# bytedance/particle-sfm

Measured on NVIDIA H100. Metric: global_ba_observations_per_sec, higher is better.
Workload: dtype f64

## Files before the change

particle-sfm_b200/csrc/ba_kernels.cuh:

```cuda
#pragma once
#include "psfm_common.cuh"

namespace psfm {
namespace ba {

constexpr int NVL = 18;
constexpr int NVI = 9;
constexpr int NREP = 32;

struct TileCtx {
  const int* tile_start;
  const int* tile_pt;
  const int* pt_ptr;
  const int* obs_img;
  const int* obs_pt;
  const unsigned short* obs_lseg;
  const unsigned short* obs_lpt;
  const double2* obs_xy;
  const unsigned short* tile_perm;
  const int* cseg_ptr;
  const int* cseg_img;
  const unsigned short* cseg_off;
  const int* img_cam;
  int F, P, M, C, T;
// ... 409 lines not shown
}

template <int TILE, bool ROT>
__global__ void __launch_bounds__(TILE, (TILE == 256 ? 3 : 1)) k_linearize(const TileCtx tc, const LinArgs a) {
  extern __shared__ __align__(16) unsigned char smem_raw[];
  TileSmem<TILE> sm;
  sm.carve(smem_raw, 18, 3, tc.cap_ns, tc.cap_np);
  const TileInfo ti = tile_header(tc);
  const int tid = threadIdx.x;
  const bool act = tid < ti.n;
  const size_t i = (size_t)ti.base + tid;
  int ls = 0, lp = 0;
  double2 xy = make_double2(0.0, 0.0);
  if (act) {
    ls = __ldg(tc.obs_lseg + i);
    lp = __ldg(tc.obs_lpt + i);
    xy = tc.obs_xy[i];
  }
  tile_fill_smem<TILE>(tc, sm, ti, a.pose16, nullptr, a.X, nullptr, nullptr, true);
  linearize_tile<TILE, ROT>(tc, a, sm, ti, act, ls, lp, xy, blockIdx.x);
}


struct PtsArgs {
  const double* hpp;
  const double* gp;
  const double* wk;
  const double* scale_p;
  double radius, min_diag, max_diag;
  int intr;
  int P;
  double* ht;
  double* wt;
  double* acc_intr;
  double* acc_fail;
  double* gmax;
};

__global__ void __launch_bounds__(256) k_point_blocks(const PtsArgs a) {
  __shared__ double sred[9 * 32];
  const int p = blockIdx.x * 256 + threadIdx.x;
  double gm = 0.0, fail = 0.0;
  double ci[9];
#pragma unroll
  for (int k = 0; k < 9; ++k) ci[k] = 0.0;
  if (p < a.P) {
    const size_t P = a.P;
    const double s0 = a.scale_p[3 * (size_t)p], s1 = a.scale_p[3 * (size_t)p + 1], s2 = a.scale_p[3 * (size_t)p + 2];
    double h00 = a.hpp[p] * s0 * s0, h01 = a.hpp[P + p] * s0 * s1, h02 = a.hpp[2 * P + p] * s0 * s2,
           h11 = a.hpp[3 * P + p] * s1 * s1, h12 = a.hpp[4 * P + p] * s1 * s2, h22 = a.hpp[5 * P + p] * s2 * s2;
    const double g0 = a.gp[p], g1 = a.gp[P + p], g2 = a.gp[2 * P + p];
    h00 += fmin(fmax(h00, a.min_diag), a.max_diag) / a.radius;
    h11 += fmin(fmax(h11, a.min_diag), a.max_diag) / a.radius;
    h22 += fmin(fmax(h22, a.min_diag), a.max_diag) / a.radius;
    bool bad = !(h00 > 0.0);
    const double l00 = sqrt(h00);
    const double l10 = h01 / l00, l20 = h02 / l00;
    double d = h11 - l10 * l10;
    bad |= !(d > 0.0);
    const double l11 = sqrt(d);
    const double l21 = (h12 - l20 * l10) / l11;
    d = h22 - l20 * l20 - l21 * l21;
    bad |= !(d > 0.0);
    const double l22 = sqrt(d);
    const double i00 = 1.0 / l00, i11 = 1.0 / l11, i22 = 1.0 / l22;
    const double i10 = -l10 * i00 * i11;
    const double i21 = -l21 * i11 * i22;
    const double i20 = -(l20 * i00 + l21 * i10) * i22;
    double v00 = i00 * i00 + i10 * i10 + i20 * i20, v01 = i10 * i11 + i20 * i21, v02 = i20 * i22,
           v11 = i11 * i11 + i21 * i21, v12 = i21 * i22, v22 = i22 * i22;
    if (bad) { fail = 1.0; v00 = v11 = v22 = 1.0; v01 = v02 = v12 = 0.0; }
    v00 *= s0 * s0; v01 *= s0 * s1; v02 *= s0 * s2; v11 *= s1 * s1; v12 *= s1 * s2; v22 *= s2 * s2;
    a.ht[p] = v00; a.ht[P + p] = v01; a.ht[2 * P + p] = v02;
    a.ht[3 * P + p] = v11; a.ht[4 * P + p] = v12; a.ht[5 * P + p] = v22;
    const double w0 = v00 * g0 + v01 * g1 + v02 * g2;
    const double w1 = v01 * g0 + v11 * g1 + v12 * g2;
    const double w2 = v02 * g0 + v12 * g1 + v22 * g2;
    a.wt[p] = w0; a.wt[P + p] = w1; a.wt[2 * P + p] = w2;
    gm = fmax(fmax(fabs(g0), fabs(g1)), fabs(g2));
    if (a.intr >= 1) {
      double W[3][3], WH[3][3];
      for (int j = 0; j < 3; ++j)
        for (int k = 0; k < 3; ++k) W[j][k] = (j < a.intr) ? a.wk[(size_t)(3 * j + k) * P + p] : 0.0;
      for (int j = 0; j < 3; ++j) {
        WH[j][0] = W[j][0] * v00 + W[j][1] * v01 + W[j][2] * v02;
        WH[j][1] = W[j][0] * v01 + W[j][1] * v11 + W[j][2] * v12;
        WH[j][2] = W[j][0] * v02 + W[j][1] * v12 + W[j][2] * v22;
      }
      int c = 0;
      for (int j = 0; j < 3; ++j)
        for (int k = j; k < 3; ++k) ci[c++] = -(WH[j][0] * W[k][0] + WH[j][1] * W[k][1] + WH[j][2] * W[k][2]);
      for (int j = 0; j < 3; ++j) ci[6 + j] = -(W[j][0] * w0 + W[j][1] * w1 + W[j][2] * w2);
    }
  }
  const double m = block_max(gm, sred);
  if (threadIdx.x == 0 && m > 0.0) atomic_max_nonneg(a.gmax, m);
  const double f = block_sum(fail, sred);
  if (threadIdx.x == 0 && f > 0.0) atomicAdd(a.acc_fail, f);
  if (a.intr >= 1) {
    const double s = block_sum_multi<9>(ci, sred);
    if (threadIdx.x < 9) atomicAdd(a.acc_intr + threadIdx.x, s);
  }
}

// ... 340 lines not shown
```

particle-sfm_b200/csrc/ba_schur_explicit.cuh:

```cuda
#pragma once
#include <cooperative_groups.h>
#include <cub/cub.cuh>

#include "ba_kernels.cuh"
#include "ba_tile_pipe.cuh"

namespace psfm {
namespace ba {

constexpr int NVX = 21;
constexpr int NVX2 = 27;


struct SwArgs {
  Lin L;
  const double* pose16;
  const double* X;
  const double* ht;
  const double* wk;
  const double* K;
  double* W;
  double* WH;
  double* acc_cam;
  size_t rep_stride;
// ... 122 lines not shown
    for (int k = 0; k < 36; ++k) acc[k] = 0.0;
    for (int e = rg.x; e < rg.y; ++e) {
      const unsigned int u = __ldg(a.entries + e);
      const size_t i = base + (u >> 16), j = base + (u & 0xffffu);
      const double2* wh = reinterpret_cast<const double2*>(a.WH + 18 * i);
      const double2* wj = reinterpret_cast<const double2*>(a.W + 18 * j);
      double A[18], B[18];
#pragma unroll
      for (int k = 0; k < 9; ++k) {
        const double2 x = __ldg(wh + k), y = __ldg(wj + k);
        A[2 * k] = x.x; A[2 * k + 1] = x.y;
        B[2 * k] = y.x; B[2 * k + 1] = y.y;
      }
#pragma unroll
      for (int r = 0; r < 6; ++r)
#pragma unroll
        for (int c = 0; c < 6; ++c)
          acc[6 * r + c] += A[3 * r] * B[3 * c] + A[3 * r + 1] * B[3 * c + 1] + A[3 * r + 2] * B[3 * c + 2];
    }
    double* dst = band + (size_t)__ldg(a.task_slot + q) * 36;
#pragma unroll
    for (int k = 0; k < 36; ++k)
      if (acc[k] != 0.0) atomicAdd(dst + k, acc[k]);
  }
}


constexpr int PS = 18;

struct StArgs {
  Lin L;
  const double* pose16;
  const double* X;
  const double* ht;
  const double* wt;
  const double* wk;
  const double* K;
  double* acc_cam;
  size_t rep_stride;
  int intr;
  const unsigned int* entries;
  const int* task_slot;
  const int2* task_rng;
  const int* tile_task;
  double* Sband;
  size_t band_stride;
  int nrep_mask;
  int span;
  const unsigned char* tile_dense;
};

enum : unsigned char { TILE_PAIRS_LOOP = 0, TILE_PAIRS_DENSE = 1, TILE_PAIRS_DENSE_DUP = 2 };

__host__ __device__ inline int dense_z_kb2(int np) { return (3 * np + 7) >> 3; }
__host__ __device__ inline int dense_z_rb(int ns) { return (6 * ns + 15) >> 4; }
__host__ __device__ inline size_t dense_z_doubles(int ns, int np) { return (size_t)dense_z_rb(ns) * dense_z_kb2(np) * 128; }

__device__ __forceinline__ void dmma_16x8x4(double (&d)[4], double a0, double a1, double b) {
  asm("mma.sync.aligned.m16n8k4.row.col.f64.f64.f64.f64 {%0,%1,%2,%3}, {%4,%5}, {%6}, {%0,%1,%2,%3};"
      : "+d"(d[0]), "+d"(d[1]), "+d"(d[2]), "+d"(d[3])
      : "d"(a0), "d"(a1), "d"(b));
}

__device__ __forceinline__ bool chol3(const double (&h)[6], double (&l)[6]) {
  const double d0 = h[0];
  l[0] = sqrt(d0);
  l[1] = h[1] / l[0];
  l[3] = h[2] / l[0];
  const double d1 = h[3] - l[1] * l[1];
  l[2] = sqrt(d1);
  l[4] = (h[4] - l[3] * l[1]) / l[2];
  const double d2 = h[5] - l[3] * l[3] - l[4] * l[4];
  l[5] = sqrt(d2);
  auto ok = [](double d) { return d > 0.0 && !isinf(d); };
  return ok(d0) && ok(d1) && ok(d2);
}

template <int TILE>
__device__ __forceinline__ void dense_pairs_mma(const double* __restrict__ zf, const int* __restrict__ cimg, int ns, int np,
                                                double* __restrict__ band, int span) {
  const int lane = threadIdx.x & 31, warp = threadIdx.x >> 5;
  const int R = 6 * ns, RB = dense_z_rb(ns), KB2 = dense_z_kb2(np);
  const int nblk = RB * (RB + 1) / 2;
  const double2* z2 = reinterpret_cast<const double2*>(zf);
  for (int blk = warp; blk < nblk; blk += TILE / 32) {
    int I = 0, rem = blk;
    while (rem >= RB - I) { rem -= RB - I; ++I; }
    const int J = I + rem;
    const double2* pa0 = z2 + (size_t)(2 * I) * KB2 * 32 + (lane ^ ((2 * I) & 7));
    const double2* pa1 = z2 + (size_t)(2 * I + 1) * KB2 * 32 + (lane ^ ((2 * I + 1) & 7));
    const double2* pb0 = z2 + (size_t)(2 * J) * KB2 * 32 + (lane ^ ((2 * J) & 7));
    const double2* pb1 = z2 + (size_t)(2 * J + 1) * KB2 * 32 + (lane ^ ((2 * J + 1) & 7));
    double acc[2][4];
#pragma unroll
    for (int h = 0; h < 2; ++h)
#pragma unroll
      for (int e = 0; e < 4; ++e) acc[h][e] = 0.0;
#pragma unroll 2
    for (int k = 0; k < KB2; ++k) {
      const double2 a0 = pa0[32 * k], a1 = pa1[32 * k], b0 = pb0[32 * k], b1 = pb1[32 * k];
      dmma_16x8x4(acc[0], a0.x, a1.x, b0.x);
      dmma_16x8x4(acc[1], a0.x, a1.x, b1.x);
      dmma_16x8x4(acc[0], a0.y, a1.y, b0.y);
      dmma_16x8x4(acc[1], a0.y, a1.y, b1.y);
    }
#pragma unroll
    for (int h = 0; h < 2; ++h)
#pragma unroll
// ... 6 lines not shown
        const int ia = cimg[sr], d = cimg[sc] - ia;
        if (d > span) continue;
        double* blkp = band + ((size_t)ia * (span + 1) + d) * 36;
        atomicAdd(blkp + 6 * (r - 6 * sr) + (c - 6 * sc), v);
        if (sr == sc && (r >> 3) < (c >> 3)) atomicAdd(blkp + 6 * (c - 6 * sc) + (r - 6 * sr), v);
      }
  }
}

template <int TILE, bool ROT>
__device__ __forceinline__ void schur_tile_body(const TileCtx& tc, const StArgs& a, TileSmem<TILE>& sm, const TileInfo& ti,
                                                const bool act, const int ls, const int lp, const double a00, const double a02,
                                                const double a12, const int rep, const int t0, const int nt) {
  const int tid = threadIdx.x;
  const double inv_f = (a.intr >= 1) ? 1.0 / __ldg(a.K) : 0.0;
  const unsigned char mode = __ldg(a.tile_dense + rep);
  constexpr int lpt = 2;
  const int nq = 2 * max(nt, 0);
  auto lane_task = [&](int q, int& tq, int& par) -> bool {
    par = q & 1; tq = q >> 1;
    return q < nq;
  };
  int tq_f, par_f;
  const bool valid_f = lane_task(tid, tq_f, par_f);
  int2 rg_f = make_int2(0, 0);
  int slot_f = 0;
  if (valid_f) { rg_f = __ldg(a.task_rng + t0 + tq_f); slot_f = __ldg(a.task_slot + t0 + tq_f); }
  double* sv = sm.sv + tid;
#pragma unroll
  for (int k = 0; k < NVX2; ++k) sv[k * PSFM_SVS] = 0.0;
  double rec[18];
#pragma unroll
  for (int k = 0; k < 18; ++k) rec[k] = 0.0;
  bool pivot_bad = false;
  if (act) {
    ObsGeom g;
    load_geom<TILE>(sm, ls, lp, g);
    const int cnp = sm.cap_np;
    double hv[6], wkp[3], wh[3];
#pragma unroll
    for (int k = 0; k < 6; ++k) hv[k] = sm.prow(3 + k)[lp];
    if (mode != TILE_PAIRS_LOOP) {
      double lh[6];
      pivot_bad = !chol3(hv, lh);
    }
#pragma unroll
    for (int k = 0; k < 3; ++k) { wkp[k] = sm.prow(9 + k)[lp]; wh[k] = sm.prow(12 + k)[lp]; }
    double jp[2][3], jc[2][6], Q[2][3];
#pragma unroll
    for (int k = 0; k < 3; ++k) {
      jp[0][k] = a00 * g.R[k] + a02 * g.R[6 + k];
      jp[1][k] = a00 * g.R[3 + k] + a12 * g.R[6 + k];
    }
#pragma unroll
    for (int m = 0; m < 2; ++m) {
      Q[m][0] = jp[m][0] * hv[0] + jp[m][1] * hv[1] + jp[m][2] * hv[2];
      Q[m][1] = jp[m][0] * hv[1] + jp[m][1] * hv[3] + jp[m][2] * hv[4];
      Q[m][2] = jp[m][0] * hv[2] + jp[m][1] * hv[4] + jp[m][2] * hv[5];
    }
    if (ROT) {
      jc[0][0] = 2.0 * a02 * g.w[1]; jc[0][1] = 2.0 * (a00 * g.w[2] - a02 * g.w[0]); jc[0][2] = -2.0 * a00 * g.w[1];
      jc[1][0] = 2.0 * (a12 * g.w[1] - a00 * g.w[2]); jc[1][1] = -2.0 * a12 * g.w[0]; jc[1][2] = 2.0 * a00 * g.w[0];
    } else {
#pragma unroll
      for (int k = 0; k < 3; ++k) { jc[0][k] = 0.0; jc[1][k] = 0.0; }
    }
    jc[0][3] = a00; jc[0][4] = 0.0; jc[0][5] = a02;
    jc[1][3] = 0.0; jc[1][4] = a00; jc[1][5] = a12;
    rec[0] = a00; rec[1] = a02; rec[2] = a12;
#pragma unroll
    for (int k = 0; k < 3; ++k) { rec[3 + k] = g.w[k]; rec[6 + k] = Q[0][k]; rec[9 + k] = Q[1][k]; rec[12 + k] = jp[0][k]; rec[15 + k] = jp[1][k]; }
    if (ROT) {
#pragma unroll
      for (int r = 0; r < 3; ++r)
#pragma unroll
        for (int c = 0; c < 3; ++c) sv[(3 * r + c) * PSFM_SVS] = jc[0][r] * jc[0][3 + c] + jc[1][r] * jc[1][3 + c];
    }
    if (a.intr >= 1) {
      const double zf = (g.w[2] + g.tz) * inv_f;
      const double jf0 = -a02 * zf, jf1 = -a12 * zf;
      const double qk0 = Q[0][0] * wkp[0] + Q[0][1] * wkp[1] + Q[0][2] * wkp[2];
      const double qk1 = Q[1][0] * wkp[0] + Q[1][1] * wkp[1] + Q[1][2] * wkp[2];
#pragma unroll
      for (int r = 0; r < 6; ++r) {
        sv[(9 + r) * PSFM_SVS] = jc[0][r] * jf0 + jc[1][r] * jf1;
        sv[(15 + r) * PSFM_SVS] = -(jc[0][r] * qk0 + jc[1][r] * qk1);
      }
    }
    const double pw0 = jp[0][0] * wh[0] + jp[0][1] * wh[1] + jp[0][2] * wh[2];
    const double pw1 = jp[1][0] * wh[0] + jp[1][1] * wh[1] + jp[1][2] * wh[2];
#pragma unroll
    for (int r = (ROT ? 0 : 3); r < 6; ++r) sv[(21 + r) * PSFM_SVS] = -(jc[0][r] * pw0 + jc[1][r] * pw1);
  }
  const bool dense = !__syncthreads_or(pivot_bad) && mode != TILE_PAIRS_LOOP;
  {
    double* dst = a.acc_cam + (size_t)(rep & (NREP - 1)) * a.rep_stride;
    tile_reduce_images<TILE>(sm, ti, NVX2, [&](int k, int img, double acc) {
      if (acc != 0.0) atomicAdd(dst + (size_t)img * NVX2 + k, acc);
    });
  }
  __syncthreads();
  double* band = a.Sband + (size_t)(rep & a.nrep_mask) * a.band_stride;
  if (dense) {
    double* zf = sm.sv;
    const int nz2 = (int)(dense_z_doubles(ti.ns, ti.np) / 2);
    for (int k = tid; k < nz2; k += TILE) reinterpret_cast<double2*>(zf)[k] = make_double2(0.0, 0.0);
    __syncthreads();
    if (act) {
      double hv[6], lh[6];
#pragma unroll
      for (int k = 0; k < 6; ++k) hv[k] = sm.prow(3 + k)[lp];
      chol3(hv, lh);
      const double w0 = rec[3], w1 = rec[4], w2 = rec[5];
      double jl[2][3], jc[2][6];
#pragma unroll
      for (int m = 0; m < 2; ++m) {
        const double p0 = rec[12 + 3 * m], p1 = rec[13 + 3 * m], p2 = rec[14 + 3 * m];
        jl[m][0] = p0 * lh[0] + p1 * lh[1] + p2 * lh[3];
        jl[m][1] = p1 * lh[2] + p2 * lh[4];
        jl[m][2] = p2 * lh[5];
      }
      if (ROT) {
        jc[0][0] = 2.0 * a02 * w1; jc[0][1] = 2.0 * (a00 * w2 - a02 * w0); jc[0][2] = -2.0 * a00 * w1;
        jc[1][0] = 2.0 * (a12 * w1 - a00 * w2); jc[1][1] = -2.0 * a12 * w0; jc[1][2] = 2.0 * a00 * w0;
      }
      jc[0][3] = a00; jc[0][4] = 0.0; jc[0][5] = a02;
      jc[1][3] = 0.0; jc[1][4] = a00; jc[1][5] = a12;
      const int KB2 = dense_z_kb2(ti.np);
#pragma unroll
      for (int r = (ROT ? 0 : 3); r < 6; ++r)
#pragma unroll
        for (int k = 0; k < 3; ++k) {
          const int row = 6 * ls + r, col = 3 * lp + k;
          const int q = row >> 3;
          double* z = zf + (((q * KB2 + (col >> 3)) * 32 + (((row & 7) * 4 + (col & 3)) ^ (q & 7))) * 2 + ((col >> 2) & 1));
          const double v = jc[0][r] * jl[0][k] + jc[1][r] * jl[1][k];
          if (mode == TILE_PAIRS_DENSE_DUP) atomicAdd(z, v); else *z = v;
        }
    }
    __syncthreads();
    dense_pairs_mma<TILE>(zf, sm.cimg, ti.ns, ti.np, band, a.span);
    return;
  }
  unsigned int uf0 = 0u, uf1 = 0u, uf2 = 0u;
  {
    const int e = rg_f.x + par_f;
    if (e < rg_f.y) uf0 = __ldg(a.entries + e);
    if (e + lpt < rg_f.y) uf1 = __ldg(a.entries + e + lpt);
    if (e + 2 * lpt < rg_f.y) uf2 = __ldg(a.entries + e + 2 * lpt);
  }
  double* srec = sm.sv;
  if (act) {
    double2* o = reinterpret_cast<double2*>(srec + (size_t)tid * PS);
#pragma unroll
    for (int k = 0; k < 9; ++k) o[k] = make_double2(rec[2 * k], rec[2 * k + 1]);
  }
  __syncthreads();
  for (int q0 = 0; q0 < nq; q0 += TILE) {
    int tq = tq_f, par = par_f, e0 = rg_f.x, e1 = rg_f.y, slot = slot_f;
    bool valid = valid_f;
    unsigned int u0 = uf0, u1 = uf1, u2 = uf2;
    if (q0 > 0) {
      valid = lane_task(q0 + tid, tq, par);
      e0 = e1 = 0; u0 = u1 = u2 = 0u;
      if (valid) {
        const int2 rg = __ldg(a.task_rng + t0 + tq);
        slot = __ldg(a.task_slot + t0 + tq);
        e0 = rg.x; e1 = rg.y;
        const int e = e0 + par;
        if (e < e1) u0 = __ldg(a.entries + e);
// ... 63 lines not shown
      for (int r = 0; r < 3; ++r)
#pragma unroll
        for (int c = 0; c < 3; ++c) { acc[6 * r + c] *= 4.0; acc[6 * r + 3 + c] *= 2.0; acc[6 * (3 + r) + c] *= 2.0; }
    }
    double* dst = band + (size_t)slot * 36;
#pragma unroll
    for (int i = 0; i < 18; ++i) {
      const double mine = par ? acc[18 + i] : acc[i];
      const double x = par ? acc[i] : acc[18 + i];
      const double v = mine + __shfl_xor_sync(0xffffffffu, x, 1);
      if (valid && (ROT || v != 0.0)) atomicAdd(dst + 18 * par + i, v);
    }
  }
}

template <int TILE, bool ROT>
__global__ void __launch_bounds__(TILE, (TILE == 256 ? 2 : 1)) k_schur_tile(const TileCtx tc, const StArgs a) {
  extern __shared__ __align__(16) unsigned char smem_raw[];
  TileSmem<TILE> sm;
  sm.carve(smem_raw, NVX2, 15, tc.cap_ns, tc.cap_np);
  const TileInfo ti = tile_header(tc);
  const int tid = threadIdx.x;
  const bool act = tid < ti.n;
  const size_t M = tc.M;
  const size_t i = (size_t)ti.base + tid;
  int ls = 0, lp = 0;
  double a00 = 0, a02 = 0, a12 = 0;
  if (act) {
    ls = __ldg(tc.obs_lseg + i);
    lp = __ldg(tc.obs_lpt + i);
    a00 = a.L.a[i]; a02 = a.L.a[M + i]; a12 = a.L.a[2 * M + i];
  }
  const int t0 = __ldg(a.tile_task + blockIdx.x), nt = __ldg(a.tile_task + blockIdx.x + 1) - t0;
  tile_fill_smem<TILE>(tc, sm, ti, a.pose16, nullptr, a.X, a.ht, a.wk, true, a.wt);
  schur_tile_body<TILE, ROT>(tc, a, sm, ti, act, ls, lp, a00, a02, a12, blockIdx.x, t0, nt);
}

template <int TILE, bool ROT>
__global__ void __launch_bounds__(TILE, (TILE == 256 ? 2 : 1)) k_schur_tile_p(const TileCtx tc, const PipeSrc ps, const StArgs a) {
  extern __shared__ __align__(16) unsigned char smem_raw[];
  __shared__ __align__(16) int4 hdr_ring[4][2];
  __shared__ __align__(8) unsigned long long bars[2];
  const int cns = tc.cap_ns, cnp = tc.cap_np;
  const size_t sb = PipeStage<TILE>::bytes(false, true, 15, cns, cnp);
  TileSmem<TILE> sm;
  sm.cap_ns = cns; sm.cap_np = cnp;
  sm.sv = reinterpret_cast<double*>(smem_raw + 2 * sb);
  sm.sw = nullptr; sm.sred = nullptr; sm.sx = nullptr;
  pipe_run<TILE>(tc, ps, smem_raw, hdr_ring, bars, 15, cns, cnp, [&](const TileInfo& ti, const PipeStage<TILE>& s, int tile) {
    view_stage<TILE>(sm, s);
    const int tid = threadIdx.x;
    const bool act = tid < ti.n;
    int ls = 0, lp = 0;
    double a00 = 0, a02 = 0, a12 = 0;
    if (act) { ls = s.lseg[tid]; lp = s.lpt[tid]; a00 = s.a0[tid]; a02 = s.a1[tid]; a12 = s.a2[tid]; }
    const int t0 = __ldg(a.tile_task + tile), nt = __ldg(a.tile_task + tile + 1) - t0;
    schur_tile_body<TILE, ROT>(tc, a, sm, ti, act, ls, lp, a00, a02, a12, tile, t0, nt);
  });
}

template <int TILE>
inline size_t pipe_smem_schur_tile(int cns, int cnp) {
  return 2 * PipeStage<TILE>::bytes(false, true, 15, cns, cnp) + sizeof(double) * NVX2 * (TILE + 1);
}


__global__ void k_pair_fill_tile(const int* pt_ptr, const int* obs_pt, const int* obs_img, const int* ptr, int M,
// ... 378 lines not shown
```

particle-sfm_b200/csrc/ba_solver.cu:

```cuda
#include <algorithm>
#include <chrono>
#include <cstdlib>
#include <cmath>
#include <mutex>
#include <thread>
#include <vector>

#include "ba_small_kernels.cuh"
#include "ba_structure.cuh"
#include "ba_schur_explicit.cuh"
#include "ba_band_chol.cuh"
#include "ba_refine.cuh"
#include "dist.cuh"

namespace psfm {
namespace ba {

struct EventPool {
  std::vector<cudaEvent_t> ev;
  size_t used = 0;
  cudaEvent_t get() {
    if (used == ev.size()) {
      cudaEvent_t e;
      PSFM_CUDA(cudaEventCreate(&e));
// ... 88 lines not shown
  int flags_world = 1;
  std::vector<double> h_qvec, h_tvec, h_K;
  DBuf<int> d_tile_start, d_tile_pt, d_pt_ptr, d_obs_img, d_obs_pt, d_cseg_ptr, d_cseg_img, d_img_cam;
  DBuf<unsigned short> d_tile_perm, d_cseg_off, d_obs_lseg, d_obs_lpt;
  DBuf<int> d_obs_orig;
  DBuf<double2> d_obs_xy;
  bool pipe = false;
  int sm_count = 0;
  DBuf<int4> d_tile_hdr;
  DBuf<int> d_pstart_rel, d_cseg_off32;
  DBuf<double> d_seg_pose;
  DBuf<unsigned char> d_active;
  DBuf<double> d_pose[2], d_X[2], d_K[2];
  int cur = 0;
  DBuf<double> d_r, d_a, d_pose16, d_xs, d_hpp, d_gp, d_wk, d_hinv, d_w, d_scale_c, d_scale_p;
  DBuf<double> d_lin, d_prep, d_step, d_rep, d_gmax, d_x2, d_Dc2, d_Minv, d_rhs, d_x, d_rv, d_p, d_z, d_y, d_zero;
  DBuf<double> d_camrep, d_yrep;
  bool pairs_ready = false;
  bool pb_fresh = false;
  double pb_radius = 0.0;
  int bw = 0;
  long long npairs = 0;
  DBuf<int> d_cholfail;
  DBuf<unsigned int> d_cholbar;
  DBuf<double> d_cholLp, d_cholLd;
  DBuf<double> d_W, d_WH, d_xcamrep, d_S;
  bool fused = false;
  int span = 0, ntasks = 0, band_nrep = 1;
  size_t band_n = 0;
  DBuf<unsigned int> d_tentries;
  DBuf<int> d_task_slot, d_tile_task;
  DBuf<int2> d_task_rng;
  DBuf<double> d_xband, d_bandrep;
  DBuf<unsigned char> d_tile_pairs;
  int ndense = 0;
  bool band_chol = false;
  BandWork bwk;
  DBuf<PcgState> d_pcg;
  HostScalars* hs = nullptr;
  double* pin_state = nullptr;
  size_t pin_state_bytes = 0, hs_bytes = 0;
  cudaStream_t stream = nullptr;
  EventPool events;
  std::vector<std::pair<cudaEvent_t, cudaEvent_t>> ev_lin, ev_sp, ev_sw, ev_pairs, ev_chol;

  TileCtx tc() const {
    TileCtx t;
    t.tile_start = d_tile_start.p; t.tile_pt = d_tile_pt.p; t.pt_ptr = d_pt_ptr.p;
    t.obs_img = d_obs_img.p; t.obs_pt = d_obs_pt.p; t.obs_xy = d_obs_xy.p;
    t.obs_lseg = d_obs_lseg.p; t.obs_lpt = d_obs_lpt.p; t.cap_ns = cap_ns; t.cap_np = cap_np;
    t.tile_perm = d_tile_perm.p; t.cseg_ptr = d_cseg_ptr.p; t.cseg_img = d_cseg_img.p;
    t.cseg_off = d_cseg_off.p; t.img_cam = d_img_cam.p;
    t.F = F; t.P = P; t.M = M; t.C = C; t.T = T;
    return t;
  }
  ~psfm_ba_solver() {
    if (stream) cudaStreamSynchronize(stream);
    g_pinned.release(hs, hs_bytes);
    g_pinned.release(pin_state, pin_state_bytes);
  }
};

namespace {

double now_s() {
  return std::chrono::duration<double>(std::chrono::steady_clock::now().time_since_epoch()).count();
// ... 448 lines not shown
  a.pose16 = S->d_pose16.p; a.X = S->d_X[S->cur].p; a.K = S->d_K[S->cur].p;
  a.loss.type = c.o.loss_function_type; a.loss.a = c.o.loss_function_scale;
  a.intr = c.intr;
  a.L = lin_of(S);
  a.hpp = S->d_hpp.p; a.gp = S->d_gp.p; a.wk = S->d_wk.p;
  a.acc_cam = S->d_camrep.p; a.rep_stride = (size_t)S->F * NVL; a.acc_intr = S->d_lin.p + (size_t)S->F * NVL;
  a.acc_cost = S->d_lin.p + (size_t)S->F * NVL + (size_t)S->C * NVI;
  cudaEvent_t e0 = nullptr, e1 = nullptr;
  const size_t pipe_smem = S->tile == 256 ? pipe_smem_linearize<256>(S->cap_ns, S->cap_np) : pipe_smem_linearize<512>(S->cap_ns, S->cap_np);
  if (pipe_ok(S, pipe_smem)) {
    k_seg_pose<<<grid_for(12 * (size_t)S->nseg), 256, 0, S->stream>>>(S->d_cseg_img.p, S->d_pose16.p, S->nseg, S->d_seg_pose.p);
    PSFM_LAUNCH_CHECK();
  }
  if (timed) { e0 = S->events.get(); e1 = S->events.get(); PSFM_CUDA(cudaEventRecord(e0, S->stream)); }
  if (pipe_ok(S, pipe_smem)) {
    PipeSrc ps = pipe_src(S);
    ps.obs_xy = S->d_obs_xy.p;
    PSFM_PIPE_LAUNCH(k_linearize_p, pipe_smem, S, c.rot, ps, a);
  } else {
    PSFM_TILE_LAUNCH(k_linearize, 18, 3, S, c.rot, a);
  }
  if (timed) { PSFM_CUDA(cudaEventRecord(e1, S->stream)); S->ev_lin.push_back({e0, e1}); }
  fold_replicas(S, S->d_lin.p, S->d_camrep.p, (size_t)S->F * NVL, nullptr, nullptr);
  dist::allreduce_sum(S->d_lin.p, S->d_lin.n, S->stream);
}

void do_point_blocks(psfm_ba_solver* S, const RunCfg& c, double radius) {
  if (S->P == 0) return;
  PtsArgs a;
  a.hpp = S->d_hpp.p; a.gp = S->d_gp.p; a.wk = S->d_wk.p; a.scale_p = S->d_scale_p.p;
  a.radius = radius; a.min_diag = c.o.min_lm_diagonal; a.max_diag = c.o.max_lm_diagonal;
  a.intr = c.intr; a.P = S->P;
  a.ht = S->d_hinv.p; a.wt = S->d_w.p;
  a.acc_intr = S->d_prep.p + (size_t)S->F * NVL;
  a.acc_fail = S->d_prep.p + (size_t)S->F * NVL + (size_t)S->C * NVI;
  a.gmax = S->d_gmax.p;
  k_point_blocks<<<(S->P + 255) / 256, 256, 0, S->stream>>>(a);
  PSFM_LAUNCH_CHECK();
}

void do_cam_gmax(psfm_ba_solver* S) {
  const int n = S->F + S->C;
  k_cam_gmax<<<(n + 127) / 128, 128, 0, S->stream>>>(S->d_lin.p, S->d_lin.p + (size_t)S->F * NVL,
                                                     S->d_active.p, S->d_pose[S->cur].p, S->F, S->C, S->d_gmax.p);
  PSFM_LAUNCH_CHECK();
}

void cam_finalize(psfm_ba_solver* S, const RunCfg& c, double radius, bool fused) {
  CamFinArgs f;
  f.lin_cam = S->d_lin.p; f.lin_intr = S->d_lin.p + (size_t)S->F * NVL;
  if (fused) { f.prep_cam = S->d_xband.p; f.prep_stride = NVX2; f.prep_goff = 21; f.prep_blocks = 0; }
  else { f.prep_cam = S->d_prep.p; f.prep_stride = NVL; f.prep_goff = 12; f.prep_blocks = 1; }
  f.prep_intr = S->d_prep.p + (size_t)S->F * NVL;
  f.active = S->d_active.p; f.scale_c = S->d_scale_c.p; f.radius = radius; f.min_diag = c.o.min_lm_diagonal; f.max_diag = c.o.max_lm_diagonal;
  f.F = S->F; f.C = S->C; f.Dc2 = S->d_Dc2.p; f.Minv = S->d_Minv.p; f.rhs = S->d_rhs.p;
  k_cam_finalize<<<(S->NB + 127) / 128, 128, 0, S->stream>>>(f);
  PSFM_LAUNCH_CHECK();
}

void do_reduced_setup(psfm_ba_solver* S, const RunCfg& c, double radius, bool fused_explicit = false) {
  if (!(S->pb_fresh && S->pb_radius == radius)) {
    S->d_prep.zero(S->stream);
    do_point_blocks(S, c, radius);
  }
  S->pb_fresh = false;
  if (fused_explicit) {
// ... 170 lines not shown
  PSFM_CUDA(cudaMemsetAsync(cnt.p + M, 0, sizeof(int), st));
  if (M) {
    k_pair_count<<<grid_for(M), 256, 0, st>>>(S->d_pt_ptr.p, S->d_obs_pt.p, S->d_obs_img.p, M, cnt.p);
    PSFM_LAUNCH_CHECK();
    k_point_span<<<grid_for(S->P), 256, 0, st>>>(S->d_pt_ptr.p, S->d_obs_img.p, S->P, span.p);
    PSFM_LAUNCH_CHECK();
  }
  DBuf<long long> ptr64;
  ptr64.alloc((size_t)M + 1, st);
  {
    size_t need = 0;
    cub::DeviceScan::ExclusiveSum(nullptr, need, cnt.p, ptr64.p, M + 1, st);
    DBuf<unsigned char> tmp; tmp.alloc(need + 256, st);
    cub::DeviceScan::ExclusiveSum(tmp.p, need, cnt.p, ptr64.p, M + 1, st);
    long long total = 0; int h_span = 0;
    PSFM_CUDA(cudaMemcpyAsync(&total, ptr64.p + M, sizeof(long long), cudaMemcpyDeviceToHost, st));
    PSFM_CUDA(cudaMemcpyAsync(&h_span, span.p, sizeof(int), cudaMemcpyDeviceToHost, st));
    PSFM_CUDA(cudaStreamSynchronize(st));
    S->npairs = total;
    h_span = (int)(reduce_over_ranks(st, h_span, dist::allreduce_max) + 0.5);
    S->bw = 6 * h_span + 5;
  }
  if (reduce_over_ranks(st, S->npairs >= (1ll << 31) ? 1.0 : 0.0, dist::allreduce_max) > 0.5) {
    set_error("too many observation pairs for the explicit Schur complement");
    throw CudaFail{PSFM_ERR_UNSUPPORTED};
  }
  S->span = (S->bw - 5) / 6;
  {
    const size_t smem256 = TileSmem<256>::bytes(NVX2, 15, S->cap_ns, S->cap_np), smem512 = TileSmem<512>::bytes(NVX2, 15, S->cap_ns, S->cap_np);
    const size_t smem = S->tile == 256 ? smem256 : smem512;
    S->fused = smem <= 227 * 1024 && !getenv("PSFM_SCHUR_UNFUSED");
  }
  S->fused = reduce_over_ranks(st, S->fused ? 0.0 : 1.0, dist::allreduce_max) < 0.5;
  S->band_n = (size_t)F * (S->span + 1) * 36;
  if (M == 0) {
    S->ntasks = 0; S->ndense = 0; S->band_nrep = 1;
    S->d_xband.alloc((size_t)F * NVX2 + S->band_n, st);
    S->d_bandrep.alloc(S->band_n, st); S->d_bandrep.zero(st);
    S->d_xcamrep.alloc((size_t)NREP * F * NVX2, st); S->d_xcamrep.zero(st);
    S->d_cholfail.alloc(1, st);
    setup_band_chol(S);
    PSFM_CUDA(cudaStreamSynchronize(st));
    S->pairs_ready = true;
    return;
  }
  const size_t NPr = (size_t)S->npairs;
  DBuf<int> ptr32; ptr32.alloc((size_t)M + 1, st);
  {
    size_t need = 0;
    cub::DeviceScan::ExclusiveSum(nullptr, need, cnt.p, ptr32.p, M + 1, st);
    DBuf<unsigned char> tmp; tmp.alloc(need + 256, st);
    cub::DeviceScan::ExclusiveSum(tmp.p, need, cnt.p, ptr32.p, M + 1, st);
  }
  const int T = S->T;
  int fb = 1; while ((1 << fb) < F) ++fb;
  DBuf<unsigned long long> k64, k64_out, uk64;
  DBuf<unsigned int> v32;
  k64.alloc(NPr, st); k64_out.alloc(NPr, st); v32.alloc(NPr, st); S->d_tentries.alloc(NPr, st);
  k_pair_fill_tile<<<grid_for(M), 256, 0, st>>>(S->d_pt_ptr.p, S->d_obs_pt.p, S->d_obs_img.p, ptr32.p, M,
                                                 S->d_tile_start.p, T, fb, k64.p, v32.p);
  PSFM_LAUNCH_CHECK();
  {
    DBuf<int> seg; seg.alloc((size_t)T + 1, st);
    k_tile_entry_offsets<<<grid_for((size_t)T + 1), 256, 0, st>>>(S->d_tile_start.p, ptr32.p, T, seg.p); PSFM_LAUNCH_CHECK();
    size_t need = 0;
    cub::DeviceSegmentedRadixSort::SortPairs(nullptr, need, k64.p, k64_out.p, v32.p, S->d_tentries.p, (int)NPr, T, seg.p, seg.p + 1, 0, 2 * fb, st);
// ... 91 lines not shown
    PSFM_LAUNCH_CHECK();
  }
  { cudaEvent_t e = S->events.get(); PSFM_CUDA(cudaEventRecord(e, st)); S->ev_chol.back().second = e; }
}

void launch_band_cholesky(psfm_ba_solver* S) {
  cudaStream_t st = S->stream;
  const BandPlan& pl = S->bwk.pl;
  BandAsmArgs2 b;
  b.Sband = S->d_xband.p + (size_t)S->F * NVX2;
  b.lin_cam = S->d_lin.p; b.lin_intr = S->d_lin.p + (size_t)S->F * NVL;
  b.prep_intr = S->d_prep.p + (size_t)S->F * NVL;
  b.xcam = S->d_xband.p; b.xstride = NVX2;
  b.scale_c = S->d_scale_c.p; b.Dc2 = S->d_Dc2.p; b.rhs = S->d_rhs.p; b.active = S->d_active.p;
  b.F = S->F; b.span = S->span; b.pl = pl;
  b.Ab = S->bwk.ab(0); b.Ab1 = S->bwk.ab(1); b.C4 = S->bwk.C4.p; b.fail = S->d_cholfail.p;
  k_band_assemble<<<grid_for((size_t)(pl.rows[0] + pl.rows[1]) * pl.RS), 256, 0, st>>>(b);
  PSFM_LAUNCH_CHECK();
  band_chol_launch(S->bwk.args(S->d_x.p, S->NS, S->d_cholfail.p), st);
  { cudaEvent_t e = S->events.get(); PSFM_CUDA(cudaEventRecord(e, st)); S->ev_chol.back().second = e; }
}


void do_explicit_solve(psfm_ba_solver* S, const RunCfg& c, double radius) {
  cudaStream_t st = S->stream;
  const size_t nx = (size_t)S->F * NVX2;
  auto mark = [&](std::vector<std::pair<cudaEvent_t, cudaEvent_t>>& v, bool begin) {
    cudaEvent_t e = S->events.get();
    PSFM_CUDA(cudaEventRecord(e, st));
    if (begin) v.push_back({e, nullptr}); else v.back().second = e;
  };
  if (S->fused) {
    StArgs w;
    w.L = lin_of(S); w.pose16 = S->d_pose16.p; w.X = S->d_X[S->cur].p; w.ht = S->d_hinv.p; w.wt = S->d_w.p; w.wk = S->d_wk.p;
    w.K = S->d_K[S->cur].p; w.acc_cam = S->d_xcamrep.p; w.rep_stride = nx; w.intr = c.intr;
    w.entries = S->d_tentries.p; w.task_slot = S->d_task_slot.p; w.task_rng = S->d_task_rng.p; w.tile_task = S->d_tile_task.p;
    w.Sband = S->d_bandrep.p; w.band_stride = S->band_n; w.nrep_mask = S->band_nrep - 1;
    w.span = S->span; w.tile_dense = S->d_tile_pairs.p;
    mark(S->ev_sw, true);
    const size_t pipe_smem = S->tile == 256 ? pipe_smem_schur_tile<256>(S->cap_ns, S->cap_np) : pipe_smem_schur_tile<512>(S->cap_ns, S->cap_np);
    if (pipe_ok(S, pipe_smem) && !getenv("PSFM_NO_PIPE_SCHUR")) {
      PipeSrc ps = pipe_src(S);
      ps.obs_a = S->d_a.p; ps.p6 = S->d_hinv.p; ps.p3a = S->d_wk.p; ps.p3b = S->d_w.p;
      PSFM_PIPE_LAUNCH(k_schur_tile_p, pipe_smem, S, c.rot, ps, w);
    } else {
      PSFM_TILE_LAUNCH(k_schur_tile, NVX2, 15, S, c.rot, w);
    }
    mark(S->ev_sw, false);
  } else {
    SwArgs w;
    w.L = lin_of(S); w.pose16 = S->d_pose16.p; w.X = S->d_X[S->cur].p; w.ht = S->d_hinv.p; w.wk = S->d_wk.p;
    w.K = S->d_K[S->cur].p; w.W = S->d_W.p; w.WH = S->d_WH.p; w.acc_cam = S->d_xcamrep.p; w.rep_stride = nx; w.intr = c.intr;
    mark(S->ev_sw, true);
    PSFM_TILE_LAUNCH(k_schur_w, NVX, 12, S, c.rot, w);
    mark(S->ev_sw, false);
    PairArgs pa;
    pa.entries = S->d_tentries.p; pa.task_slot = S->d_task_slot.p; pa.task_rng = S->d_task_rng.p; pa.tile_task = S->d_tile_task.p;
    pa.tile_start = S->d_tile_start.p; pa.W = S->d_W.p; pa.WH = S->d_WH.p;
    pa.Sband = S->d_bandrep.p; pa.band_stride = S->band_n; pa.nrep_mask = S->band_nrep - 1;
    mark(S->ev_pairs, true);
    if (S->T > 0) { k_schur_pairs<<<S->T, 128, 0, st>>>(pa); PSFM_LAUNCH_CHECK(); }
    mark(S->ev_pairs, false);
  }
  mark(S->ev_chol, true);
  k_fold_replicas2<<<grid_for(nx + S->band_n), 256, 0, st>>>(S->d_xband.p, S->d_xcamrep.p, nx, NREP, S->d_bandrep.p, S->band_n, S->band_nrep);
  PSFM_LAUNCH_CHECK();
  dist::allreduce_sum(S->d_xband.p, S->d_xband.n, st);
  if (S->fused) cam_finalize(S, c, radius, true);
  if (S->band_chol) { launch_band_cholesky(S); return; }
  S->d_S.zero(st);
  BandAsmArgs ba_;
  ba_.Sband = S->d_xband.p + nx; ba_.scale_c = S->d_scale_c.p; ba_.F = S->F; ba_.span = S->span; ba_.lda = S->NS + 1; ba_.S = S->d_S.p;
  k_schur_assemble_band<<<grid_for(S->band_n), 256, 0, st>>>(ba_); PSFM_LAUNCH_CHECK();
  AsmArgs a;
  a.lin_cam = S->d_lin.p; a.lin_intr = S->d_lin.p + (size_t)S->F * NVL;
  a.prep_intr = S->d_prep.p + (size_t)S->F * NVL; a.xcam = S->d_xband.p; a.xstride = NVX2;
// ... 752 lines not shown
```

Measured before the change: 290.2 million.

## Precompute per-point Cholesky factors so the Schur tile skips per-observation chol3

The point-block kernel now also writes the scaled inverse Cholesky factor of each point's Hessian block, plus the gradient and intrinsic coupling terms pre-multiplied by that factor. The fused Schur tile kernel reads these instead of the inverse Hessian. It forms factored Jacobians directly, so the per-observation chol3 calls, the block-wide pivot check and the recomputation of camera Jacobians in the dense pair path all go away. The cost is three extra per-point arrays written each iteration. Points whose factorisation fails now fall back to an identity-scaled factor instead of switching the tile to the loop path.

```diff
diff --git a/particle-sfm_b200/csrc/ba_kernels.cuh b/particle-sfm_b200/csrc/ba_kernels.cuh
--- a/particle-sfm_b200/csrc/ba_kernels.cuh
+++ b/particle-sfm_b200/csrc/ba_kernels.cuh
@@ -465,6 +465,9 @@
   int P;
   double* ht;
   double* wt;
+  double* gf;
+  double* gv;
+  double* gu;
   double* acc_intr;
   double* acc_fail;
   double* gmax;
@@ -503,6 +506,16 @@
     double v00 = i00 * i00 + i10 * i10 + i20 * i20, v01 = i10 * i11 + i20 * i21, v02 = i20 * i22,
            v11 = i11 * i11 + i21 * i21, v12 = i21 * i22, v22 = i22 * i22;
     if (bad) { fail = 1.0; v00 = v11 = v22 = 1.0; v01 = v02 = v12 = 0.0; }
+    if (a.gf) {
+      double f00 = s0, f01 = 0.0, f02 = 0.0, f11 = s1, f12 = 0.0, f22 = s2;
+      if (!bad) { f00 = s0 * i00; f01 = s0 * i10; f02 = s0 * i20; f11 = s1 * i11; f12 = s1 * i21; f22 = s2 * i22; }
+      a.gf[p] = f00; a.gf[P + p] = f01; a.gf[2 * P + p] = f02;
+      a.gf[3 * P + p] = f11; a.gf[4 * P + p] = f12; a.gf[5 * P + p] = f22;
+      a.gu[p] = f00 * g0; a.gu[P + p] = f01 * g0 + f11 * g1; a.gu[2 * P + p] = f02 * g0 + f12 * g1 + f22 * g2;
+      double k0 = 0.0, k1 = 0.0, k2 = 0.0;
+      if (a.intr >= 1) { k0 = a.wk[p]; k1 = a.wk[P + p]; k2 = a.wk[2 * P + p]; }
+      a.gv[p] = f00 * k0; a.gv[P + p] = f01 * k0 + f11 * k1; a.gv[2 * P + p] = f02 * k0 + f12 * k1 + f22 * k2;
+    }
     v00 *= s0 * s0; v01 *= s0 * s1; v02 *= s0 * s2; v11 *= s1 * s1; v12 *= s1 * s2; v22 *= s2 * s2;
     a.ht[p] = v00; a.ht[P + p] = v01; a.ht[2 * P + p] = v02;
     a.ht[3 * P + p] = v11; a.ht[4 * P + p] = v12; a.ht[5 * P + p] = v22;
diff --git a/particle-sfm_b200/csrc/ba_schur_explicit.cuh b/particle-sfm_b200/csrc/ba_schur_explicit.cuh
--- a/particle-sfm_b200/csrc/ba_schur_explicit.cuh
+++ b/particle-sfm_b200/csrc/ba_schur_explicit.cuh
@@ -178,9 +178,9 @@
   Lin L;
   const double* pose16;
   const double* X;
-  const double* ht;
-  const double* wt;
-  const double* wk;
+  const double* gf;
+  const double* gv;
+  const double* gu;
   const double* K;
   double* acc_cam;
   size_t rep_stride;
@@ -206,20 +206,6 @@
   asm("mma.sync.aligned.m16n8k4.row.col.f64.f64.f64.f64 {%0,%1,%2,%3}, {%4,%5}, {%6}, {%0,%1,%2,%3};"
       : "+d"(d[0]), "+d"(d[1]), "+d"(d[2]), "+d"(d[3])
       : "d"(a0), "d"(a1), "d"(b));
-}
-
-__device__ __forceinline__ bool chol3(const double (&h)[6], double (&l)[6]) {
-  const double d0 = h[0];
-  l[0] = sqrt(d0);
-  l[1] = h[1] / l[0];
-  l[3] = h[2] / l[0];
-  const double d1 = h[3] - l[1] * l[1];
-  l[2] = sqrt(d1);
-  l[4] = (h[4] - l[3] * l[1]) / l[2];
-  const double d2 = h[5] - l[3] * l[3] - l[4] * l[4];
-  l[5] = sqrt(d2);
-  auto ok = [](double d) { return d > 0.0 && !isinf(d); };
-  return ok(d0) && ok(d1) && ok(d2);
 }
 
 template <int TILE>
@@ -292,21 +278,14 @@
   double rec[18];
 #pragma unroll
   for (int k = 0; k < 18; ++k) rec[k] = 0.0;
-  bool pivot_bad = false;
   if (act) {
     ObsGeom g;
     load_geom<TILE>(sm, ls, lp, g);
     const int cnp = sm.cap_np;
-    double hv[6], wkp[3], wh[3];
-#pragma unroll
-    for (int k = 0; k < 6; ++k) hv[k] = sm.prow(3 + k)[lp];
-    if (mode != TILE_PAIRS_LOOP) {
-      double lh[6];
-      pivot_bad = !chol3(hv, lh);
-    }
-#pragma unroll
-    for (int k = 0; k < 3; ++k) { wkp[k] = sm.prow(9 + k)[lp]; wh[k] = sm.prow(12 + k)[lp]; }
-    double jp[2][3], jc[2][6], Q[2][3];
+    double gm[6];
+#pragma unroll
+    for (int k = 0; k < 6; ++k) gm[k] = sm.prow(3 + k)[lp];
+    double jp[2][3], jc[2][6], jg[2][3];
 #pragma unroll
     for (int k = 0; k < 3; ++k) {
       jp[0][k] = a00 * g.R[k] + a02 * g.R[6 + k];
@@ -314,9 +293,9 @@
     }
 #pragma unroll
     for (int m = 0; m < 2; ++m) {
-      Q[m][0] = jp[m][0] * hv[0] + jp[m][1] * hv[1] + jp[m][2] * hv[2];
-      Q[m][1] = jp[m][0] * hv[1] + jp[m][1] * hv[3] + jp[m][2] * hv[4];
-      Q[m][2] = jp[m][0] * hv[2] + jp[m][1] * hv[4] + jp[m][2] * hv[5];
+      jg[m][0] = jp[m][0] * gm[0];
+      jg[m][1] = jp[m][0] * gm[1] + jp[m][1] * gm[3];
+      jg[m][2] = jp[m][0] * gm[2] + jp[m][1] * gm[4] + jp[m][2] * gm[5];
     }
     if (ROT) {
       jc[0][0] = 2.0 * a02 * g.w[1]; jc[0][1] = 2.0 * (a00 * g.w[2] - a02 * g.w[0]); jc[0][2] = -2.0 * a00 * g.w[1];
@@ -327,9 +306,6 @@
     }
     jc[0][3] = a00; jc[0][4] = 0.0; jc[0][5] = a02;
     jc[1][3] = 0.0; jc[1][4] = a00; jc[1][5] = a12;
-    rec[0] = a00; rec[1] = a02; rec[2] = a12;
-#pragma unroll
-    for (int k = 0; k < 3; ++k) { rec[3 + k] = g.w[k]; rec[6 + k] = Q[0][k]; rec[9 + k] = Q[1][k]; rec[12 + k] = jp[0][k]; rec[15 + k] = jp[1][k]; }
     if (ROT) {
 #pragma unroll
       for (int r = 0; r < 3; ++r)
@@ -339,20 +315,38 @@
     if (a.intr >= 1) {
       const double zf = (g.w[2] + g.tz) * inv_f;
       const double jf0 = -a02 * zf, jf1 = -a12 * zf;
-      const double qk0 = Q[0][0] * wkp[0] + Q[0][1] * wkp[1] + Q[0][2] * wkp[2];
-      const double qk1 = Q[1][0] * wkp[0] + Q[1][1] * wkp[1] + Q[1][2] * wkp[2];
+      const double gk[3] = {sm.prow(9)[lp], sm.prow(10)[lp], sm.prow(11)[lp]};
+      const double qk0 = jg[0][0] * gk[0] + jg[0][1] * gk[1] + jg[0][2] * gk[2];
+      const double qk1 = jg[1][0] * gk[0] + jg[1][1] * gk[1] + jg[1][2] * gk[2];
 #pragma unroll
       for (int r = 0; r < 6; ++r) {
         sv[(9 + r) * PSFM_SVS] = jc[0][r] * jf0 + jc[1][r] * jf1;
         sv[(15 + r) * PSFM_SVS] = -(jc[0][r] * qk0 + jc[1][r] * qk1);
       }
     }
-    const double pw0 = jp[0][0] * wh[0] + jp[0][1] * wh[1] + jp[0][2] * wh[2];
-    const double pw1 = jp[1][0] * wh[0] + jp[1][1] * wh[1] + jp[1][2] * wh[2];
+    const double gg[3] = {sm.prow(12)[lp], sm.prow(13)[lp], sm.prow(14)[lp]};
+    const double pw0 = jg[0][0] * gg[0] + jg[0][1] * gg[1] + jg[0][2] * gg[2];
+    const double pw1 = jg[1][0] * gg[0] + jg[1][1] * gg[1] + jg[1][2] * gg[2];
 #pragma unroll
     for (int r = (ROT ? 0 : 3); r < 6; ++r) sv[(21 + r) * PSFM_SVS] = -(jc[0][r] * pw0 + jc[1][r] * pw1);
-  }
-  const bool dense = !__syncthreads_or(pivot_bad) && mode != TILE_PAIRS_LOOP;
+    if (mode == TILE_PAIRS_LOOP) {
+      rec[0] = a00; rec[1] = a02; rec[2] = a12;
+#pragma unroll
+      for (int m = 0; m < 2; ++m) {
+        rec[6 + 3 * m] = jg[m][0] * gm[0] + jg[m][1] * gm[1] + jg[m][2] * gm[2];
+        rec[7 + 3 * m] = jg[m][1] * gm[3] + jg[m][2] * gm[4];
+        rec[8 + 3 * m] = jg[m][2] * gm[5];
+      }
+#pragma unroll
+      for (int k = 0; k < 3; ++k) { rec[3 + k] = g.w[k]; rec[12 + k] = jp[0][k]; rec[15 + k] = jp[1][k]; }
+    } else {
+#pragma unroll
+      for (int r = 0; r < 6; ++r)
+#pragma unroll
+        for (int k = 0; k < 3; ++k) rec[3 * r + k] = jc[0][r] * jg[0][k] + jc[1][r] * jg[1][k];
+    }
+  }
+  __syncthreads();
   {
     double* dst = a.acc_cam + (size_t)(rep & (NREP - 1)) * a.rep_stride;
     tile_reduce_images<TILE>(sm, ti, NVX2, [&](int k, int img, double acc) {
@@ -361,41 +355,23 @@
   }
   __syncthreads();
   double* band = a.Sband + (size_t)(rep & a.nrep_mask) * a.band_stride;
-  if (dense) {
+  if (mode != TILE_PAIRS_LOOP) {
     double* zf = sm.sv;
-    const int nz2 = (int)(dense_z_doubles(ti.ns, ti.np) / 2);
+    const int KB2 = dense_z_kb2(ti.np), zrows = 16 * dense_z_rb(ti.ns), zcols = 8 * KB2;
+    auto zat = [&](int row, int col) -> double* {
+      const int q = row >> 3;
+      return zf + (((q * KB2 + (col >> 3)) * 32 + (((row & 7) * 4 + (col & 3)) ^ (q & 7))) * 2 + ((col >> 2) & 1));
+    };
+    const int nz2 = zrows * zcols / 2;
     for (int k = tid; k < nz2; k += TILE) reinterpret_cast<double2*>(zf)[k] = make_double2(0.0, 0.0);
     __syncthreads();
     if (act) {
-      double hv[6], lh[6];
-#pragma unroll
-      for (int k = 0; k < 6; ++k) hv[k] = sm.prow(3 + k)[lp];
-      chol3(hv, lh);
-      const double w0 = rec[3], w1 = rec[4], w2 = rec[5];
-      double jl[2][3], jc[2][6];
-#pragma unroll
-      for (int m = 0; m < 2; ++m) {
-        const double p0 = rec[12 + 3 * m], p1 = rec[13 + 3 * m], p2 = rec[14 + 3 * m];
-        jl[m][0] = p0 * lh[0] + p1 * lh[1] + p2 * lh[3];
-        jl[m][1] = p1 * lh[2] + p2 * lh[4];
-        jl[m][2] = p2 * lh[5];
-      }
-      if (ROT) {
-        jc[0][0] = 2.0 * a02 * w1; jc[0][1] = 2.0 * (a00 * w2 - a02 * w0); jc[0][2] = -2.0 * a00 * w1;
-        jc[1][0] = 2.0 * (a12 * w1 - a00 * w2); jc[1][1] = -2.0 * a12 * w0; jc[1][2] = 2.0 * a00 * w0;
-      }
-      jc[0][3] = a00; jc[0][4] = 0.0; jc[0][5] = a02;
-      jc[1][3] = 0.0; jc[1][4] = a00; jc[1][5] = a12;
-      const int KB2 = dense_z_kb2(ti.np);
-#pragma unroll
-      for (int r = (ROT ? 0 : 3); r < 6; ++r)
+#pragma unroll
+      for (int r = 0; r < 6; ++r)
 #pragma unroll
         for (int k = 0; k < 3; ++k) {
-          const int row = 6 * ls + r, col = 3 * lp + k;
-          const int q = row >> 3;
-          double* z = zf + (((q * KB2 + (col >> 3)) * 32 + (((row & 7) * 4 + (col & 3)) ^ (q & 7))) * 2 + ((col >> 2) & 1));
-          const double v = jc[0][r] * jl[0][k] + jc[1][r] * jl[1][k];
-          if (mode == TILE_PAIRS_DENSE_DUP) atomicAdd(z, v); else *z = v;
+          double* z = zat(6 * ls + r, 3 * lp + k);
+          if (mode == TILE_PAIRS_DENSE_DUP) atomicAdd(z, rec[3 * r + k]); else *z = rec[3 * r + k];
         }
     }
     __syncthreads();
@@ -525,7 +501,7 @@
     a00 = a.L.a[i]; a02 = a.L.a[M + i]; a12 = a.L.a[2 * M + i];
   }
   const int t0 = __ldg(a.tile_task + blockIdx.x), nt = __ldg(a.tile_task + blockIdx.x + 1) - t0;
-  tile_fill_smem<TILE>(tc, sm, ti, a.pose16, nullptr, a.X, a.ht, a.wk, true, a.wt);
+  tile_fill_smem<TILE>(tc, sm, ti, a.pose16, nullptr, a.X, a.gf, a.gv, true, a.gu);
   schur_tile_body<TILE, ROT>(tc, a, sm, ti, act, ls, lp, a00, a02, a12, blockIdx.x, t0, nt);
 }
 
diff --git a/particle-sfm_b200/csrc/ba_solver.cu b/particle-sfm_b200/csrc/ba_solver.cu
--- a/particle-sfm_b200/csrc/ba_solver.cu
+++ b/particle-sfm_b200/csrc/ba_solver.cu
@@ -144,6 +144,7 @@
   DBuf<int> d_task_slot, d_tile_task;
   DBuf<int2> d_task_rng;
   DBuf<double> d_xband, d_bandrep;
+  DBuf<double> d_gf, d_gv, d_gu;
   DBuf<unsigned char> d_tile_pairs;
   int ndense = 0;
   bool band_chol = false;
@@ -658,6 +659,8 @@
   a.radius = radius; a.min_diag = c.o.min_lm_diagonal; a.max_diag = c.o.max_lm_diagonal;
   a.intr = c.intr; a.P = S->P;
   a.ht = S->d_hinv.p; a.wt = S->d_w.p;
+  const bool gfac = S->pairs_ready && S->fused;
+  a.gf = gfac ? S->d_gf.p : nullptr; a.gv = S->d_gv.p; a.gu = S->d_gu.p;
   a.acc_intr = S->d_prep.p + (size_t)S->F * NVL;
   a.acc_fail = S->d_prep.p + (size_t)S->F * NVL + (size_t)S->C * NVI;
   a.gmax = S->d_gmax.p;
@@ -894,6 +897,10 @@
     S->fused = smem <= 227 * 1024 && !getenv("PSFM_SCHUR_UNFUSED");
   }
   S->fused = reduce_over_ranks(st, S->fused ? 0.0 : 1.0, dist::allreduce_max) < 0.5;
+  if (S->fused) {
+    S->d_gf.alloc(6 * (size_t)S->P, st); S->d_gv.alloc(3 * (size_t)S->P, st); S->d_gu.alloc(3 * (size_t)S->P, st);
+    S->pb_fresh = false;
+  }
   S->band_n = (size_t)F * (S->span + 1) * 36;
   if (M == 0) {
     S->ntasks = 0; S->ndense = 0; S->band_nrep = 1;
@@ -1051,7 +1058,7 @@
   };
   if (S->fused) {
     StArgs w;
-    w.L = lin_of(S); w.pose16 = S->d_pose16.p; w.X = S->d_X[S->cur].p; w.ht = S->d_hinv.p; w.wt = S->d_w.p; w.wk = S->d_wk.p;
+    w.L = lin_of(S); w.pose16 = S->d_pose16.p; w.X = S->d_X[S->cur].p; w.gf = S->d_gf.p; w.gv = S->d_gv.p; w.gu = S->d_gu.p;
     w.K = S->d_K[S->cur].p; w.acc_cam = S->d_xcamrep.p; w.rep_stride = nx; w.intr = c.intr;
     w.entries = S->d_tentries.p; w.task_slot = S->d_task_slot.p; w.task_rng = S->d_task_rng.p; w.tile_task = S->d_tile_task.p;
     w.Sband = S->d_bandrep.p; w.band_stride = S->band_n; w.nrep_mask = S->band_nrep - 1;
@@ -1060,7 +1067,7 @@
     const size_t pipe_smem = S->tile == 256 ? pipe_smem_schur_tile<256>(S->cap_ns, S->cap_np) : pipe_smem_schur_tile<512>(S->cap_ns, S->cap_np);
     if (pipe_ok(S, pipe_smem) && !getenv("PSFM_NO_PIPE_SCHUR")) {
       PipeSrc ps = pipe_src(S);
-      ps.obs_a = S->d_a.p; ps.p6 = S->d_hinv.p; ps.p3a = S->d_wk.p; ps.p3b = S->d_w.p;
+      ps.obs_a = S->d_a.p; ps.p6 = S->d_gf.p; ps.p3a = S->d_gv.p; ps.p3b = S->d_gu.p;
       PSFM_PIPE_LAUNCH(k_schur_tile_p, pipe_smem, S, c.rot, ps, w);
     } else {
       PSFM_TILE_LAUNCH(k_schur_tile, NVX2, 15, S, c.rot, w);
```

New measurement: 308.2 million, median of 6. +6.2%, better.
